# Rongjiehuang/FastDiff

Measured on AMD Instinct MI355X. Metric: real-time factor (audio-sec/wall-sec), N=4 reverse steps, 80x864 mel, higher is better.
Workload: dtype f32 results; 2-piece fp16 operands (22 bit) on fp16 MFMA, fp32 accumulate; GEMM as Winograd F(2,3); exact-fp32 twin; 1 GPU; BASELINE configs[1]: LJSpeech shape, batch=8 x 80x864 mel per GPU, N=4, HIP kernels + hipGraph sampler; batch_per_gpu=8, frames=864, reverse_steps=4, graph=True, weights=random init seed 1234 (no checkpoint offline), world_size=1, gpus_visible=1, oversubscribed=False

## Files before the change

### fastdiff_amd/csrc/fd_api.cpp

```cpp
#include <math.h>
#include <stddef.h>
#include <stdio.h>
#include <stdlib.h>
#include <string.h>

#include <algorithm>

#include "fd_kernels.h"
#include "fd_host.h"

std::string g_create_error;

static inline int gx_rows_host(int T) { return std::max(fdk_fast::gx_rows(T), fdk_fast::gw_pairs(T) * (fdk_fast::GW_ROWB / fdk_fast::GX_ROWB)); }

bool fd_prof_stamps(const fdk::Launch &L, const char *name, hipEvent_t *e0, hipEvent_t *e1)
{
    fd_context *c = L.ctx;
    if (c->profile != 1 || L.capturing) return false;
    hipEvent_t ev[2];
    for (int i = 0; i < 2; ++i) {
        if (!c->event_pool.empty()) { ev[i] = c->event_pool.back(); c->event_pool.pop_back(); }
        else if (hipEventCreate(&ev[i]) != hipSuccess) return false;
    }
    ProfEntry pe;
// ... 730 lines not shown
            int redone = resolve_pending(h, &mask);
            if (redone < 0) return redone;
        }
        if ((rc = copy_out()) != FD_OK) return rc;
    } else {
        if ((rc = enqueue_steps(h, B, T, N, mode, stream)) != FD_OK) return rc;
        if ((rc = copy_out()) != FD_OK) return rc;
    }
    h->last_B = B; h->last_T = T;
    return fd_mark_tail(h, stream);
}

int fd_sample(fd_handle h, const float *mel, int B, int T, const int *lens, const fd_step *table, int N, int ddim,
              const float *x_T, const float *z, uint64_t seed, float *out, float *seq_out, void *stream_)
{
    std::vector<unsigned long long> ids;
    std::vector<long long> offs;
    if (h) { ids.swap(h->noise_ids); offs.swap(h->noise_offs); }
    int rc = check_common(h, B, T, "fd_sample");
    if (rc != FD_OK) return rc;
    if ((rc = fd_follow_stream(h, (hipStream_t)stream_)) != FD_OK) return rc;
    if (h->gen) {
        if (!mel || !table || !out) FD_FAIL(h, FD_ERR_INVALID, "fd_sample: null pointer");
        if (N <= 0 || N > 1024) FD_FAIL(h, FD_ERR_INVALID, "fd_sample: N=%d outside 1..1024", N);
        if (!ids.empty() && (int)ids.size() != B) FD_FAIL(h, FD_ERR_INVALID, "fd_sample: fd_set_noise_streams gave %d stream ids but B=%d", (int)ids.size(), B);
        for (int b = 0; lens && b < B; ++b)
            if (lens[b] < 1 || lens[b] > T) FD_FAIL(h, FD_ERR_INVALID, "fd_sample: lens[%d] = %d outside [1, T=%d]", b, lens[b], T);
        if ((rc = fdg::sample(h, mel, B, T, lens, table, N, ddim, x_T, z, seed, ids, out, seq_out, (hipStream_t)stream_)) != FD_OK) return rc;
        ++h->ticket_counter;
        h->last_B = B; h->last_T = T;
        return fd_mark_tail(h, (hipStream_t)stream_);
    }
    const bool lazy = h->host_fallback && N >= 1 && N <= 8;
    const int Tp = bucket_frames(h, T);
    if ((rc = check_common(h, B, Tp, "fd_sample")) != FD_OK) return rc;
    const int np = (N >= 1 && N <= 1024) ? hoist_mult(h, B, Tp, N) : 1;
    const bool ws_ok = workspace_fits(h, B, Tp, np);
    fd_context::PendingCall prev;
    if (lazy && ws_ok && h->pending.active && h->pending.lazy) {
        prev = h->pending;
        h->pending.active = false;
    } else if ((rc = fd_settle(h)) != FD_OK) return rc;
    auto finish_prev = [&]() -> int {
        if (!prev.active) return FD_OK;
        unsigned mask = 0;
        const fd_context::PendingCall cur = h->pending;
        h->pending.active = false;
        const int r = resolve_call(h, prev, &mask);
        h->pending = cur;
        prev.active = false;
        return r < 0 ? r : FD_OK;
    };
    if (!mel || !table || !out) { finish_prev(); FD_FAIL(h, FD_ERR_INVALID, "fd_sample: null pointer"); }
    if (N <= 0 || N > 1024) { finish_prev(); FD_FAIL(h, FD_ERR_INVALID, "fd_sample: N=%d outside 1..1024", N); }
    if (!ids.empty() && (int)ids.size() != B) {
        finish_prev();
        FD_FAIL(h, FD_ERR_INVALID, "fd_sample: fd_set_noise_streams gave %d stream ids but B=%d", (int)ids.size(), B);
    }
    if (!offs.empty() && offs.size() != ids.size()) { finish_prev(); FD_FAIL(h, FD_ERR_INVALID, "fd_sample: noise offsets without their stream ids"); }
    for (int b = 0; lens && b < B; ++b)
        if (lens[b] < 1 || lens[b] > T) {
            finish_prev();
            FD_FAIL(h, FD_ERR_INVALID, "fd_sample: lens[%d] = %d outside [1, T=%d]", b, lens[b], T);
        }
    if ((rc = ensure_workspace(h, B, Tp, np)) != FD_OK) { finish_prev(); return rc; }
    fd_context::SampleArgs a;
    a.mel = mel; a.B = B; a.T = T; a.N = N; a.ddim = ddim;
    a.has_lens = lens != nullptr;
    if (lens) a.lens.assign(lens, lens + B);
    a.table.assign(table, table + N);
    a.x_T = x_T; a.z = z; a.seed = seed; a.out = out; a.seq_out = seq_out; a.stream = (hipStream_t)stream_;
    a.ids.swap(ids);
    a.offs.swap(offs);
    const long long ticket = ++h->ticket_counter;
    h->n_pieces = h->n_pieces_redone = h->n_pieces_fp32 = 0;
    h->call_fp32_mask = 0;
    rc = sample_core(h, a, 0u, ticket);
    const int rc_prev = finish_prev();
    h->last_B = B; h->last_T = Tp;
    if (rc != FD_OK || rc_prev != FD_OK) return rc != FD_OK ? rc : rc_prev;
    if (!h->defer_check) return fd_settle(h);
    return FD_OK;
}

int64_t fd_sample_ticket(fd_handle h) { return h ? (int64_t)h->ticket_counter : FD_ERR_INVALID; }

static int ticket_redone(fd_handle h, long long ticket)
{
    for (long long t : h->redone_ring)
        if (t == ticket && t != 0) return 1;
    return 0;
}

int fd_sample_settle(fd_handle h, int64_t ticket)
{
    if (!h) return FD_ERR_INVALID;
    if (ticket <= 0 || ticket > h->ticket_counter) FD_FAIL(h, FD_ERR_INVALID, "fd_sample_settle: unknown ticket %lld", (long long)ticket);
    if (h->pending.active && h->pending.ticket <= ticket) {
        FD_HIP(h, hipSetDevice(h->device));
        unsigned mask = 0;
        const int r = resolve_pending(h, &mask);
        if (r < 0) return r;
    }
    return ticket_redone(h, ticket);
}

int fd_sample_check(fd_handle h)
{
    if (!h) return FD_ERR_INVALID;
    if (!h->pending.active) return 0;
    FD_HIP(h, hipSetDevice(h->device));
    unsigned mask = 0;
    return resolve_pending(h, &mask);
}

int fd_set_noise_streams(fd_handle h, const uint64_t *stream_ids, int B)
{
    if (!h || B < 0 || (B > 0 && !stream_ids)) return FD_ERR_INVALID;
    h->noise_ids.assign(stream_ids, stream_ids + B);
    h->noise_offs.clear();
    return FD_OK;
}

int fd_set_option(fd_handle h, const char *key, const char *value)
{
    if (!h || !key || !value) return FD_ERR_INVALID;
    {
        const int rcs = fd_settle(h);
        if (rcs != FD_OK) return rcs;
    }
    const std::string k(key), v(value);
    static const char *stage_names[ST_COUNT] = {"embed", "first", "dblock", "kp_front", "kp_gemm", "convt", "lvc", "final"};
    auto parse_mode = [&](bool &dst) -> int {
        if (v == "fast") dst = true;
        else if (v == "naive") dst = false;
        else FD_FAIL(h, FD_ERR_INVALID, "fd_set_option: %s expects fast|naive, got '%s'", key, value);
        return FD_OK;
    };
    if (k == "kernels") {
        bool m = true;
        int rc = parse_mode(m);
        if (rc != FD_OK) return rc;
        for (int i = 0; i < ST_COUNT; ++i) h->mode.fast[i] = m;
        return FD_OK;
    }
    if (k.compare(0, 8, "kernels.") == 0) {
        for (int i = 0; i < ST_COUNT; ++i)
            if (k.substr(8) == stage_names[i]) return parse_mode(h->mode.fast[i]);
        FD_FAIL(h, FD_ERR_INVALID, "fd_set_option: unknown stage '%s'", key);
    }
    static const struct { const char *key, *a, *b; void (*set)(fd_context *, bool); } choices[] = {
        {"gemm", "f16x2", "fp32", [](fd_context *c, bool a) { c->mode.gemm_f16 = a; }},
        {"gemm_form", "winograd", "direct", [](fd_context *c, bool a) { c->mode.gemm_wino = a; }},
        {"lvc", "f16x2", "fp32", [](fd_context *c, bool a) { c->mode.lvc_f16 = a; }},
        {"conv", "f16x2", "fp32", [](fd_context *c, bool a) { c->mode.conv_f16 = a; }},
        {"lvc_h8", "mfma", "valu", [](fd_context *c, bool a) { c->mode.lvc_h8_mfma = a; }},
        {"fallback", "graph", "host", [](fd_context *c, bool a) { c->host_fallback = !a; }},
        {"lvc_dx", "gather", "copy", [](fd_context *c, bool a) { c->lvc_dx_gather = a; }},
        {"mel", "pwg", "tacotron", [](fd_context *c, bool a) { c->mel_variant = a ? MEL_PWG : MEL_TACOTRON; }},
    };
    for (const auto &ch : choices) {
        if (k != ch.key) continue;
        if (v != ch.a && v != ch.b) FD_FAIL(h, FD_ERR_INVALID, "fd_set_option: %s expects %s|%s, got '%s'", key, ch.a, ch.b, value);
        ch.set(h, v == ch.a);
        return FD_OK;
    }
    const bool on = (v == "1" || v == "true" || v == "on");
    if (k == "fuse_final") { h->mode.fuse_final = on; return FD_OK; }
    if (k == "fuse_up") { h->mode.fuse_up = on; return FD_OK; }
    if (k == "fuse_advance") { h->mode.fuse_advance = on; return FD_OK; }
    if (k == "embed_cache") { h->embed_cache = on; return FD_OK; }
    if (k == "hoist") {
        if (v == "auto") h->hoist_mode = 1;
        else if (v == "on") h->hoist_mode = 2;
        else if (v == "off") h->hoist_mode = 0;
        else FD_FAIL(h, FD_ERR_INVALID, "fd_set_option: hoist expects auto|on|off, got '%s'", value);
        return FD_OK;
    }
    if (k == "graph") { h->use_graph = on; return FD_OK; }
    if (k == "defer_check") { h->defer_check = on; return FD_OK; }
    if (k == "t_bucket" || k == "graph_cache") {
        char *end = nullptr;
        const long n = strtol(value, &end, 10);
        if (end == value || *end != 0 || n < 0 || n > 65536 || (k == "graph_cache" && n < 1))
            FD_FAIL(h, FD_ERR_INVALID, "fd_set_option: %s expects an integer (t_bucket: frames, 0 = exact T; graph_cache: graphs kept, >= 1), got '%s'", key, value);
        if (k == "t_bucket") h->t_bucket = (int)n;
        else h->max_graphs = (int)n;
        return FD_OK;
    }
    if (k == "profile") { h->profile = (v == "events") ? 2 : (on ? 1 : 0); return FD_OK; }
    if (k == "taps") { h->mode.keep_taps = on; return FD_OK; }
    FD_FAIL(h, FD_ERR_INVALID, "fd_set_option: unknown option '%s'", key);
}

}
```

### fastdiff_amd/csrc/fd_internal.h

```cpp
#pragma once
#include <hip/hip_runtime.h>
#include <hip/hip_ext.h>
#include <stdint.h>
#include <string.h>
#include <map>
#include <string>
#include <vector>

#include "../../include/fastdiff_hip.h"
#include "../../include/fastdiff_hip_ext.h"
#include "../../include/fastdiff_hip_train.h"

namespace fd {
constexpr int C = 32;
constexpr int COND = 80;
constexpr int HID = 64;
constexpr int NBLK = 3;
constexpr int LAYERS = 4;
constexpr int HOPT = 256;
constexpr int E_IN = 128, E_MID = 512, E_OUT = 512;
constexpr int KLAYER = 2 * C * C * 3;
constexpr int KW = KLAYER * LAYERS;
constexpr int KB = 2 * C * LAYERS;
constexpr int KREC = KW + KB;
__host__ __device__ constexpr int ratio(int n) { return n == 2 ? 4 : 8; }
__host__ __device__ constexpr int hop(int n) { return n == 0 ? 8 : (n == 1 ? 64 : 256); }
__host__ __device__ constexpr int down_factor(int d) { return d == 0 ? 4 : 8; }

__host__ __device__ inline int kernel_row(int out) { return (out & 15) + 16 * (out >> 5); }
__host__ __device__ inline int kernel_tile(int out) { return (out & 31) >> 4; }
__host__ __device__ inline int kernel_index(int layer, int in, int out, int tap)
{
    const int kk = tap * C + in, kg = kk >> 4, g = (kk >> 3) & 1, e = kk & 7;
    const int mt = kernel_tile(out), lane = kernel_row(out) + 32 * g;
    return layer * KLAYER + ((mt * 6 + kg) * 64 + lane) * 8 + e;
}
__host__ __device__ inline int bias_index(int layer, int out) { return KW + layer * 64 + kernel_tile(out) * 32 + kernel_row(out); }
}

struct ConvW {
    const float *w = nullptr;
    const float *b = nullptr;
};

struct DevWeights {
    ConvW first, final_;
    struct { ConvW res, conv[3]; } down[fd::NBLK];
    struct { ConvW fc_t, up, kp_in, kp_res[6], kc, bc, convs[fd::LAYERS]; } blk[fd::NBLK];
    const float *fc_t1_T = nullptr, *fc_t1_b = nullptr, *fc_t2_T = nullptr, *fc_t2_b = nullptr;
    const float *fc_t_T[fd::NBLK] = {}, *fc_t_b[fd::NBLK] = {};
    const float *embed_table = nullptr;
    const float *down_pack[fd::NBLK][4] = {};
    const uint16_t *down_h2[fd::NBLK][4] = {};
    bool dblock_f16_ok = false;
    const float *lvc_conv_pack[fd::NBLK][fd::LAYERS] = {};
    const uint16_t *lvc_conv_h2[fd::NBLK][fd::LAYERS] = {};
    const uint16_t *lvc_conv_h16[fd::LAYERS] = {};
    bool lvc_f16_ok = false;
    const float *kp_in_pack[fd::NBLK] = {};
    const float *kp_res_pack[fd::NBLK][6] = {};
    const uint16_t *kp_in_h2[fd::NBLK] = {};
    const uint16_t *kp_res_h2[fd::NBLK][6] = {};
    bool kpf_f16_ok = false;
    const float *gemm_pack[fd::NBLK] = {};
    const float *gemm_bias[fd::NBLK] = {};
    const uint16_t *gemm_h2_pack[fd::NBLK] = {};
    bool gemm_f16_ok = false;
    const uint16_t *gemm_w_pack[fd::NBLK] = {};
    bool gemm_w_ok = false;
    const float *up_pack[fd::NBLK] = {};
    const uint16_t *up_h2[fd::NBLK] = {};
    bool convt_f16_ok = false;
    const float *final_fuse = nullptr;
    const int *kc_perm = nullptr;
    const int *bc_perm = nullptr;
};

struct StepParams {
    fd_step table[1024];
    const float *z;
    float *seq;
    unsigned long long seed;
    int n_steps;
    int ddim;
    int step_idx;
    int l4;
    const unsigned long long *uids;
    int l4_io;
    long long n4_io;
    const long long *offs4;
};

enum Stage { ST_EMBED = 0, ST_FIRST, ST_DBLOCK, ST_KP_FRONT, ST_KP_GEMM, ST_CONVT, ST_LVC, ST_FINAL, ST_COUNT };

struct StepMode {
    bool fast[ST_COUNT] = {true, true, true, true, true, true, true, true};
    bool gemm_f16 = true;
    bool gemm_wino = true;
    bool lvc_f16 = true;
    bool conv_f16 = true;
    bool lvc_h8_mfma = true;
    bool fuse_final = true;
    bool fuse_up = true;
    bool fuse_advance = true;
    bool keep_taps = false;
    unsigned fp32_mask = 0;
    bool inline_fallback = true;
    bool ragged = false;
    int hoist_np = 1;
    bool hoist_chunk = false;

    bool operator==(const StepMode &o) const
    {
        for (int i = 0; i < ST_COUNT; ++i)
            if (fast[i] != o.fast[i]) return false;
        return gemm_f16 == o.gemm_f16 && gemm_wino == o.gemm_wino && lvc_f16 == o.lvc_f16 && conv_f16 == o.conv_f16 &&
               lvc_h8_mfma == o.lvc_h8_mfma && fuse_final == o.fuse_final && fuse_up == o.fuse_up && fuse_advance == o.fuse_advance &&
               keep_taps == o.keep_taps && fp32_mask == o.fp32_mask && inline_fallback == o.inline_fallback && ragged == o.ragged &&
               hoist_np == o.hoist_np && hoist_chunk == o.hoist_chunk;
    }
};

struct Workspace {
    int B = 0;
    int64_t frames = 0;
    int64_t rows = 0;
    float *noise = nullptr;
    float *embed_h2 = nullptr;
    float *a[4] = {};
    float *kp_h0 = nullptr, *kp_hA = nullptr, *kp_hB = nullptr;
    float *kpack = nullptr;
    float *h_f16 = nullptr;
    int *lens_dev = nullptr;
    unsigned long long *uid_dev = nullptr;
    long long *off_dev = nullptr;
    float *xsave = nullptr;
    int *range_flag = nullptr;
    float *xA = nullptr, *xB = nullptr;
    float *xtap[fd::NBLK] = {};
    int64_t pframes = 0, prows = 0, plens = 0;
    float *mel_rep = nullptr;
    float *mel = nullptr;
    float *x = nullptr;
    float *eps_acc = nullptr;
    float *steps = nullptr;
    StepParams *params = nullptr;
    size_t bytes = 0;
};

struct ProfEntry { std::string name; hipEvent_t e0, e1; };
struct Scratch { float *p = nullptr; size_t bytes = 0; };

struct MelTables {
    const float *tab = nullptr;
    const int *fb_lo = nullptr, *fb_n = nullptr, *fb_off = nullptr;
    const float *fb_w = nullptr;
};
enum MelVariant { MEL_PWG = 0, MEL_TACOTRON = 1, MEL_VARIANTS = 2 };

struct FoldedParam { std::vector<float> w, b; };
struct WeightImage {
    std::vector<char> bytes;
    std::vector<std::pair<const void **, size_t>> fields;
    template <class T> void add(const T *&dst, const std::vector<T> &v)
    {
        const size_t off = (bytes.size() + 255) & ~(size_t)255;
        bytes.resize(off + v.size() * sizeof(T));
        memcpy(bytes.data() + off, v.data(), v.size() * sizeof(T));
        fields.push_back({reinterpret_cast<const void **>(&dst), off});
    }
};
namespace fdg {
struct Net;
int validate(const fd_config &c, std::string &why);
int create(fd_context *c);
void destroy(fd_context *c);
int hop_total(const fd_context *c);
int pack_weights(fd_context *c, const std::map<std::string, FoldedParam> &f, WeightImage &img);
int forward(fd_context *c, const float *x, const float *mel, const float *steps, int B, int T, const int *lens, float *eps_out, hipStream_t stream);
int sample(fd_context *c, const float *mel, int B, int T, const int *lens, const fd_step *table, int N, int ddim, const float *x_T, const float *z,
           unsigned long long seed, const std::vector<unsigned long long> &ids, float *out, float *seq_out, hipStream_t stream);
}

struct fd_context {
    fd_config cfg;
    fdg::Net *gen = nullptr;
    int device = 0;
    int num_cus = 256;
    std::string err;
    bool committed = false;
    StepMode mode;
    bool use_graph = true;
    int profile = 0;
    std::vector<unsigned long long> noise_ids;
    std::vector<long long> noise_offs;
    bool host_fallback = true;
    std::map<std::string, std::pair<std::vector<int64_t>, std::vector<float>>> raw;
    void *weight_arena = nullptr;
    size_t weight_bytes = 0;
    DevWeights w;
    void *refresh_dev = nullptr;
    size_t refresh_dev_bytes = 0;
    unsigned *refresh_bad = nullptr;
    hipEvent_t refresh_done = nullptr;
    bool refresh_pending = false;
    long long n_refreshes = 0, n_refresh_graph_drops = 0;
    Workspace ws;
    bool lvc_dx_gather = true;
    std::vector<float> embed_t;
    int embed_B = 0;
    bool embed_valid = false;
    bool embed_cache = true;
    MelTables mel[MEL_VARIANTS];
    int mel_variant = MEL_PWG;
    std::vector<float> mel_bank[MEL_VARIANTS];
    bool mel_bank_user[MEL_VARIANTS] = {false, false};
    std::vector<void *> mel_allocs;
    int last_B = 0, last_T = 0;
    hipStream_t cap_stream = nullptr;
    hipStream_t last_stream = nullptr;
    bool have_last_stream = false;
    hipEvent_t ev_switch = nullptr;
    bool tail_marked = false;
    int hoist_mode = 1;
    struct StepGraph { int B, T, steps; StepMode mode; hipGraph_t graph; hipGraphExec_t exec; unsigned long long last_use; };
    std::vector<StepGraph> graphs;
    unsigned long long graph_clock = 0;
    struct RetiredGraph { hipGraph_t graph; hipGraphExec_t exec; hipEvent_t done; };
    std::vector<RetiredGraph> retired;
    int max_graphs = 64;
    int t_bucket = 32;
    long long n_graph_captures = 0, n_graph_hits = 0, n_graph_evictions = 0;
    bool defer_check = false;
    static constexpr int STAGE_SLOTS = 8;
    struct StageSlot { char *host = nullptr; size_t cap = 0; hipEvent_t done = nullptr; };
    StageSlot stage[STAGE_SLOTS];
    unsigned stage_next = 0;
    struct SampleArgs {
        const float *mel = nullptr;
        int B = 0, T = 0, N = 0, ddim = 0;
        bool has_lens = false;
        std::vector<int> lens;
        std::vector<fd_step> table;
        const float *x_T = nullptr, *z = nullptr;
        unsigned long long seed = 0;
        float *out = nullptr, *seq_out = nullptr;
        hipStream_t stream = nullptr;
        std::vector<unsigned long long> ids;
        std::vector<long long> offs;
    };
    struct PendingCall {
        bool active = false;
        bool lazy = false;
        int slot = 0;
        long long ticket = 0;
        int B = 0, T = 0, N = 0, first = 0, count = 0;
        int T_io = 0;
        float *out = nullptr;
        hipStream_t stream = nullptr;
        StepMode mode;
        SampleArgs args;
    } pending;
    long long ticket_counter = 0;
    long long n_pieces = 0, n_pieces_redone = 0, n_pieces_fp32 = 0, n_calls_redone = 0;
    unsigned call_fp32_mask = 0;
    long long redone_ring[16] = {};
    unsigned redone_next = 0;
    int *flags_host = nullptr;
    hipEvent_t flags_done = nullptr, flags_done2 = nullptr;
// ... 104 lines not shown
```

### fastdiff_amd/csrc/fd_kernels.h

```cpp
#pragma once
#include "fd_internal.h"

namespace fdk_fast {
constexpr int GX_CT = 4;
constexpr int GX_ROWB = 2 * 128;
constexpr int GW_PAIRS = 32;
constexpr int GW_ROWB = 1024;
__host__ __device__ inline int gx_rows(int T) { return ((T + GX_CT * 32 - 1) / (GX_CT * 32)) * (GX_CT * 32) + 2; }
__host__ __device__ inline int gw_pairs(int T) { return ((T + 2 * GW_PAIRS - 1) / (2 * GW_PAIRS)) * GW_PAIRS; }
}

namespace fdk {
hipError_t naive_first_conv(const Launch &L, const StepIO &io, int B, int T);
hipError_t naive_dblock(const Launch &L, int d, int B, int T);
hipError_t naive_kp_front(const Launch &L, const StepIO &io, int B, int T);
hipError_t naive_kp_gemm(const Launch &L, int B, int T);
hipError_t naive_convt(const Launch &L, int n, const float *x_in, float *x_out, int B, int Lin);
hipError_t naive_lvc_layer(const Launch &L, int n, int layer, float *x, const float *skip, float *y, int B, int T);
hipError_t naive_final_eps(const Launch &L, const float *x32, float *eps, int B, int T);
hipError_t naive_update(const Launch &L, float *x, const float *eps, int64_t n);
hipError_t fast_first_conv(const Launch &L, const StepIO &io, int B, int T);
hipError_t fast_dblock(const Launch &L, int d, int B, int T, const float *audio);
hipError_t fast_kp_front(const Launch &L, const StepIO &io, int B, int T);
hipError_t fast_kp_gemm(const Launch &L, int B, int T);
hipError_t fast_convt(const Launch &L, int n, const float *x_in, float *x_out, int B, int Lin);
hipError_t fast_lvc_layer(const Launch &L, const StepIO &io, int n, int layer, const float *x_in, const float *skip, float *x_out, int B, int T,
                          bool up = false);
hipError_t fast_final(const Launch &L, const StepIO &io, const float *x32, int B, int T);
bool lvc_op_needs_scratch(int Cin, int Cout, int ks, int hop);
hipError_t lvc_op_forward(const Launch &L, const float *x, const float *K, const float *bias, float *out, int B, int Cin, int Cout, int ks,
                          int T, int hop, float *scratch, int64_t kbs = 0, bool frames = false, int64_t bbs = 0);
hipError_t lvc_op_backward(const Launch &L, const float *x, const float *K, const float *dout, float *dx, float *dK, float *dbias, int B,
                           int Cin, int Cout, int ks, int T, int hop, float *scratch, int64_t kbs = 0, int64_t dkbs = 0, bool frames = false,
                           int64_t dbbs = 0);
hipError_t gate_forward(const Launch &L, const float *x, const float *y, float *out, int B, int C, int64_t len);
hipError_t gate_backward(const Launch &L, const float *y, const float *dout, float *dy, int B, int C, int64_t len);
hipError_t fan_pick(const Launch &L, const float *x, float *out, int rows, int64_t len, int f);
hipError_t fan_sum(const Launch &L, const float *const g[4], const float *gp, float *dx, int rows, int64_t len, int f);
bool kconv_supported(int M, int T);
size_t kconv_scratch_floats(int B, int M, int T);
bool kconv_frames_supported(int M, int T);
bool kconv_act_supported(int M, int T);
hipError_t kconv_forward(const Launch &L, const float *h, const float *W, const float *bias, float *out, int B, int M, int T, bool frames = false,
                         float post = 1.0f);
hipError_t kconv_backward(const Launch &L, const float *h, const float *W, const float *dout, float *dh, float *dW, float *dbias, int B, int M,
                          int T, float *scratch, bool frames = false, const float *y = nullptr, float post = 1.0f, float in_slope = 1.0f);
size_t kconv_w_multi_scratch_floats(int n, int B, int M);
hipError_t kconv_backward_w_multi(const Launch &L, int n, const float *const *h, const float *const *dout, const float *const *y, float post, int B,
                                  int M, int T, float *const *dW, float *const *dbias, float *scratch);
hipError_t kconv_forward_multi(const Launch &L, int n, const float *const *h, const float *const *W, const float *const *bias, float *const *out, int B,
                               int M, int T, float post);
size_t kconv_x_multi_scratch_floats(int n, int B, int M, int T);
hipError_t kconv_backward_x_multi(const Launch &L, int n, const float *const *h, const float *const *W, const float *const *y, const float *const *dout,
                                  float *const *dh, int B, int M, int T, float post, float in_slope, float *scratch);
hipError_t input_conv_forward_multi(const Launch &L, int n, const float *const *x, const float *const *w, const float *const *bias, float *const *out,
                                    int B, int T, float post);
size_t input_conv_multi_scratch_floats(int n, int B);
hipError_t input_conv_backward_multi(const Launch &L, int n, const float *const *x, const float *const *w, const float *const *y, const float *const *dy,
                                     float *const *dx, float *const *dw, float *const *db, int B, int T, float post, float *scratch);
bool cconv_supported(int dil, int64_t len);
size_t cconv_scratch_floats(const Launch &L, int dil, int B, int64_t len);
hipError_t cconv_forward(const Launch &L, const float *x, const float *skip, const float *w, const float *bias, float *xs_out, float *y, int B,
                         int64_t len, int dil, float pre, float post);
hipError_t cconv_backward(const Launch &L, const float *xs, const float *y, const float *w, const float *dy, const float *gxs, float *dxs,
                          float *dw, float *db, int B, int64_t len, int dil, float pre, float post, float *scratch);
size_t conv7_scratch_floats(const Launch &L, int B, int64_t len);
hipError_t conv7_forward(const Launch &L, int which, const float *x, const float *w, const float *bias, float *y, int B, int64_t len);
hipError_t conv7_backward(const Launch &L, int which, const float *x, const float *w, const float *dy, float *dx, float *dw, float *db, int B,
                          int64_t len, float *scratch);
size_t convt_scratch_floats(const Launch &L, int r, int B, int64_t len_in);
hipError_t convt_forward(const Launch &L, const float *x, const float *w, const float *bias, float *y, int B, int64_t len_in, int r);
hipError_t convt_backward(const Launch &L, const float *x, const float *w, const float *dy, float *dx, float *dw, float *db, int B, int64_t len_in,
                          int r, float *scratch);
hipError_t weight_norm_multi(const Launch &L, const fd_wn_item *items, int n, bool backward);
size_t step_scratch_floats(int64_t blocks);
int64_t mse_blocks(int64_t n);
int64_t adamw_blocks(const fd_adamw_item *items, int n);
hipError_t train_draw(const Launch &L, const float *x0, const float *alpha, int T_train, int B, int64_t len, uint64_t seed,
                      const fd_train_state *state, uint64_t iter_host, float *x_t, float *z, float *steps);
hipError_t train_collate(const Launch &L, const float *wav_arena, const float *mel_arena, const int64_t *frame_off, int64_t n_items, int hop,
                         int F, int B, uint64_t seed, const fd_train_state *state, uint64_t iter_host, int rank, int world, float *wavs,
                         float *mels, int64_t *picked);
hipError_t eval_collate(const Launch &L, const float *wav_arena, const float *mel_arena, const int64_t *frame_off, int64_t n_items, int hop,
                        int F, int B, uint64_t seed, const fd_train_state *state, uint64_t iter_host, float *wavs, float *mels, int64_t *picked);
int64_t item_distance_blocks(int64_t n);
hipError_t item_distance(const Launch &L, const float *a, const float *b, int B, int64_t n, int kind, float *out, float *scratch);
hipError_t eval_accumulate(const Launch &L, const float *values, const float *steps, const int64_t *picked, int B, int T_train, int bins,
                           fd_eval_state *acc, float *item_out, fd_train_state *advance);
hipError_t mse_forward(const Launch &L, const float *eps, const float *z, int64_t n, float *loss, fd_train_state *state, float *scratch);
hipError_t mse_backward(const Launch &L, const float *eps, const float *z, const float *dloss, int64_t n, float *deps);
hipError_t adamw_multi(const Launch &L, const fd_adamw_item *items, int n, const fd_adamw_hyper *hyper, fd_train_state *state, float *scratch);
hipError_t ema_multi(const Launch &L, const fd_ema_item *items, int n, const fd_ema_hyper *hyper, const fd_train_state *state, fd_ema_state *ema);
size_t bandpool_scratch_floats(int B, int64_t L, bool backward);
hipError_t bandpool_forward(const Launch &L_, const float *x, const float *W, const float *bias, int B, int64_t L, float *feat, float *scratch);
hipError_t bandpool_backward(const Launch &L_, const float *x, const float *W, const float *bias, const float *dfeat, int B, int64_t L, float *dW,
                             float *db, float *scratch);
hipError_t npred_head_forward(const Launch &L_, const float *feat, const float *beta_next, const float *delta2, int R, const float *W1,
                              const float *b1, const float *W2, const float *b2, int B, float *beta_hat, float *ratio);
hipError_t npred_head_backward(const Launch &L_, const float *feat, const float *beta_next, const float *delta2, const float *W1, const float *b1,
                               const float *W2, const float *b2, const float *dbeta_hat, int B, float *dW1, float *db1, float *dW2, float *db2,
                               float *dfeat);
hipError_t phi_draw(const Launch &L_, const float *x0, const float *alpha, int T_train, int tau, int B, int64_t len, uint64_t seed,
                    const fd_train_state *state, uint64_t iter_host, float *x_t, float *z, float *steps, float *beta_nxt, float *delta,
                    float *delta2);
int64_t phi_residual_blocks(int64_t len);
hipError_t phi_residual_forward(const Launch &L_, const float *eps, const float *z, const float *delta, const float *beta_hat, int B, int64_t len,
                                float *m, float *s, float *scratch);
hipError_t sched_init(const Launch &L_, fd_sched_state *state, float betaN, float alphaN);
hipError_t sched_begin(const Launch &L_, fd_sched_state *state, const float *beta_hat, int n_hat, double rho, const float *alpha, int T_train,
                       int ddim, float *steps_out, int B);
hipError_t sched_update(const Launch &L_, fd_sched_state *state, float *x, const float *eps, int64_t n, float *cond_out);
}

namespace fdg {
struct ConvArgs {
    const float *x, *w, *bias;
    float *y;
    int B, Cin, Cout, K;
    int64_t Lx, Lout;
    int dil = 1, in_stride = 1;
    float pre = 1.0f, post = 1.0f;
    const float *in_add = nullptr;
    int64_t in_add_b = 0, in_add_step = 0;
    const int *step = nullptr;
    const float *res = nullptr;
    const int *lens = nullptr;
    int spf = 1;
    int rec = 0, rec_off = 0;
    const int *perm = nullptr;
    ConvArgs(const ConvW &cw, const float *x_, float *y_, int B_, int Cin_, int Cout_, int K_, int64_t L)
        : x(x_), w(cw.w), bias(cw.b), y(y_), B(B_), Cin(Cin_), Cout(Cout_), K(K_), Lx(L), Lout(L) {}
};
hipError_t conv1d(const fdk::Launch &L, const char *name, const ConvArgs &a);
hipError_t convt(const fdk::Launch &L, const char *name, const ConvW &up, const float *x, float *y, int B, int C, int r, int64_t Lin,
                 const int *lens, int spf_in);
hipError_t dblock(const fdk::Launch &L, const ConvW &res, const ConvW conv[3], const float *x, int64_t Lin, int f, float *const tmp[3],
                  float *out, int B, int C, const int *lens, int spf);
hipError_t kp_front(const fdk::Launch &L, const ConvArgs &in, const ConvW res[6], int k, float *ha, float *hb);
struct LvcArgs {
    float *x;
    const float *skip;
    float *y;
    bool packed;
    const float *kernels, *biases;
    int B, C, ks, layers, layer, hop, T;
    const int *lens;
};
hipError_t lvc_layer(const fdk::Launch &L, const ConvW &conv, const LvcArgs &a);
}
```

### fastdiff_amd/csrc/fd_kernels_kp.hip

```cpp
#include "fd_kernels_common.h"

namespace fdk_fast {

constexpr int KPF_VALID = 48, KPF_LDI = 68, KPF_LDH = 66;

struct KpFrontW {
    const float *in_pack[fd::NBLK], *in_b[fd::NBLK];
    const float *res_pack[fd::NBLK][6], *res_b[fd::NBLK][6];
};

__global__ void __launch_bounds__(256, 2) k_kp_front(const float *__restrict__ mel, float *__restrict__ hout, KpFrontW w,
                                                     const float *__restrict__ noise, const StepParams *params, int sampler,
                                                     int B, int T, const int *__restrict__ run_if, const int *__restrict__ lens)
{
    __shared__ float xin[fd::COND * KPF_LDI];
    if (run_if && *run_if == 0) return;
    __shared__ float h0[fd::HID * KPF_LDH];
    __shared__ float hA[fd::HID * KPF_LDH];
    __shared__ float hB[fd::HID * KPF_LDH];
    const int blk = blockIdx.z, b = blockIdx.y, t0 = blockIdx.x * KPF_VALID;
    const int Tb = frames_of(lens, b, T);
    if (t0 >= Tb) return;
    const int tid = threadIdx.x, lane = tid & 63, wave = tid >> 6, l31 = lane & 31, hi = lane >> 5;
    const int mt = wave & 1, nt = wave >> 1;
// ... 600 lines not shown
                have_blk = cur.blk; have_xg = cur.xg;
                __builtin_amdgcn_s_waitcnt(0x0F70);
            }
            const bool more = (i + half + 1 < n_mine);
            GX_WALK_NEXT(walk, cur, more, nxt, run, left);
            const int Tb = frames_of(lens, cur.b, T);
            const bool full = (Tb % 32 == 0) || (cur.chunk * (GX_CT * 32) + GX_CT * 32 <= Tb);
            if (half == 0) {
                if (full) gx_item<0, true>(lds, cur, more, nxt, hx, kpack, wq, bias_lo, aoff, B, T, R, wave_u, lane, Tb GX_TIMING_PASS);
                else gx_item<0, false>(lds, cur, more, nxt, hx, kpack, wq, bias_lo, aoff, B, T, R, wave_u, lane, Tb GX_TIMING_PASS);
            } else {
                if (full) gx_item<1, true>(lds, cur, more, nxt, hx, kpack, wq, bias_lo, aoff, B, T, R, wave_u, lane, Tb GX_TIMING_PASS);
                else gx_item<1, false>(lds, cur, more, nxt, hx, kpack, wq, bias_lo, aoff, B, T, R, wave_u, lane, Tb GX_TIMING_PASS);
            }
            cur = nxt;
        }
    }
#ifdef FD_GX_TIMING
    ph[6] = __builtin_amdgcn_s_memtime() - t_start;
    ph[7] = __builtin_amdgcn_s_memrealtime() - r_start;
    if (lane == 0)
        for (int k = 0; k < 8; ++k) atomicAdd((unsigned long long *)&fd_gxdbg[k], (unsigned long long)ph[k]);
#endif
}

constexpr int GW_WINB = GW_PAIRS * GW_ROWB;

__global__ void __launch_bounds__(256) k_h_wino(const float *__restrict__ h, char *__restrict__ wx, int *__restrict__ range_flag, int B, int T,
                                                int P, const int *__restrict__ lens)
{
    const int bb = blockIdx.y;
    const int e = blockIdx.x * 256 + threadIdx.x, p = e >> 3, g = e & 7;
    if (p >= P) return;
    if (range_flag[32] != 0) {
        if (e == 0 && bb == 0) atomicOr(range_flag, 1);
        return;
    }
    const int Tb = frames_of(lens, bb % B, T);
    const float *hb = h + ((int64_t)bb * fd::HID + 8 * g) * T;
    const int t1 = 2 * p;
    float d[8][4];
#pragma unroll
    for (int c = 0; c < 8; ++c) {
        const float *hc = hb + (int64_t)c * T;
        d[c][0] = (t1 - 1 >= 0 && t1 - 1 < Tb) ? hc[t1 - 1] : 0.0f;
        d[c][1] = (t1 < Tb) ? hc[t1] : 0.0f;
        d[c][2] = (t1 + 1 < Tb) ? hc[t1 + 1] : 0.0f;
        d[c][3] = (t1 + 2 < Tb) ? hc[t1 + 2] : 0.0f;
    }
    float mx = 0.0f;
    char *row = wx + ((int64_t)bb * P + p) * GW_ROWB;
    const int sw = p & 15;
#pragma unroll
    for (int j = 0; j < 4; ++j) {
        float u[8];
#pragma unroll
        for (int c = 0; c < 8; ++c) {
            u[c] = j == 0 ? d[c][0] - d[c][2] : (j == 1 ? d[c][1] + d[c][2] : (j == 2 ? d[c][2] - d[c][1] : d[c][1] - d[c][3]));
            mx = fmaxf(mx, fabsf(u[c]));
        }
        float4 ph, pl;
        split8(u, ph, pl);
        *reinterpret_cast<float4 *>(row + j * 256 + ((g ^ sw) << 4)) = ph;
        *reinterpret_cast<float4 *>(row + j * 256 + (((g + 8) ^ sw) << 4)) = pl;
    }
    if (!(mx < GX_LIMIT)) atomicOr(range_flag, 1);
}

__device__ __forceinline__ void gw_dma(const char *wx, char *lds_buf, const GxItem &it, int B, int P, int wave_u, int lane)
{
#ifndef FD_GW_NO_FETCH
    gx_window_dma<GW_WINB / 4096, false>(wx + (((int64_t)it.blk * B + it.b) * P + it.chunk * GW_PAIRS) * GW_ROWB + wave_u * 1024, lds_buf, wave_u, lane);
#endif
}

template <int BUF, bool FULL>
__device__ __forceinline__ void gw_item(char *lds, const GxItem &cur, bool more, const GxItem &nxt, const char *wx, float *kpack,
                                        const float4 (&wq)[2][16], float bias_lo, const int (&aoff)[2][4], int B, int T, int P,
                                        int wave_u, int lane, int Tb)
{
    const int l31 = lane & 31, hi = lane >> 5;
    if (more) gw_dma(wx, lds + (BUF ^ 1) * GW_WINB, nxt, B, P, wave_u, lane);
    const int t_begin = cur.chunk * (2 * GW_PAIRS);
    float *krow = kpack + (((int64_t)cur.blk * B + cur.b) * T + t_begin) * fd::KREC + (cur.xg * 4 + wave_u) * 32;
    const unsigned loff = (unsigned)(8 * hi) * (unsigned)fd::KREC + (unsigned)l31;
    const __amdgpu_buffer_rsrc_t rs = __builtin_amdgcn_make_buffer_rsrc(krow, 0, 2 * GW_PAIRS * fd::KREC * 4, 0x00020000);
    const f32x16 zero = {0.f, 0.f, 0.f, 0.f, 0.f, 0.f, 0.f, 0.f, 0.f, 0.f, 0.f, 0.f, 0.f, 0.f, 0.f, 0.f};
    const char *hb = lds + BUF * GW_WINB;
    constexpr int ORDER[4] = {1, 2, 0, 3};
    f32x16 keep, acc, lo;
#pragma unroll
    for (int r = 0; r < 16; ++r) lo[r] = bias_lo;
    float4 a1, a2;
    auto store16 = [&](int odd) {
#ifdef FD_GX_NO_STORE
        if (FULL) {
#pragma unroll
            for (int r = 0; r < 16; ++r) { const float v_ = fmaf(lo[r], GX_INV_SCALE, acc[r]); asm volatile("" :: "v"(v_)); }
            (void)rs; (void)loff;
            return;
        }
#endif
        if (FULL) {
#pragma unroll
            for (int r = 0; r < 16; ++r) {
                acc[r] = fmaf(lo[r], GX_INV_SCALE, acc[r]);
                __builtin_amdgcn_raw_buffer_store_b32(__float_as_uint(acc[r]), rs, loff * 4u, (2 * ((r & 3) + 8 * (r >> 2)) + odd) * fd::KREC * 4,
                                                      FD_GX_STORE_AUX);
            }
        } else {
#pragma unroll
            for (int r = 0; r < 16; ++r)
                if (t_begin + 2 * drow(r, hi) + odd < Tb) (krow + (2 * ((r & 3) + 8 * (r >> 2)) + odd) * fd::KREC)[loff] = fmaf(lo[r], GX_INV_SCALE, acc[r]);
        }
    };
#pragma unroll
    for (int s = 0; s < 4; ++s) {
        const int j = ORDER[s];
        a1 = *reinterpret_cast<const float4 *>(hb + aoff[0][0] + j * 256);
        a2 = *reinterpret_cast<const float4 *>(hb + aoff[1][0] + j * 256);
#pragma unroll
        for (int k4 = 0; k4 < 4; ++k4) {
            const int kg = j * 4 + k4;
            float4 n1 = a1, n2 = a2;
            if (k4 + 1 < 4) {
                n1 = *reinterpret_cast<const float4 *>(hb + aoff[0][k4 + 1] + j * 256);
                n2 = *reinterpret_cast<const float4 *>(hb + aoff[1][k4 + 1] + j * 256);
            }
            acc = mfma_f16(a1, wq[0][kg], (k4 == 0 && s == 0) ? zero : ((k4 == 0 && s == 3) ? keep : acc));
            lo = mfma_f16(a2, wq[0][kg], (k4 == 0 && s == 3) ? zero : lo);
            lo = mfma_f16(a1, wq[1][kg], lo);
            a1 = n1;
            a2 = n2;
        }
        if (s == 0) {
#pragma unroll
            for (int r = 0; r < 16; ++r) keep[r] = fmaf(lo[r], GX_INV_SCALE, acc[r]);
        } else if (s == 1) {
#pragma unroll
            for (int r = 0; r < 16; ++r) keep[r] = fmaf(2.0f, keep[r], -fmaf(lo[r], GX_INV_SCALE, acc[r]));
        } else store16(s == 3 ? 1 : 0);
    }
    if (more) {
#ifdef FD_GX_NO_STORE
        asm volatile("s_waitcnt vmcnt(0)" ::: "memory");
#else
        if (FULL) asm volatile("s_waitcnt vmcnt(32)" ::: "memory");
        else asm volatile("s_waitcnt vmcnt(0)" ::: "memory");
#endif
    }
    __builtin_amdgcn_s_barrier();
}

__global__ void __launch_bounds__(256, 2) k_kp_gemm_w(const char *__restrict__ wx , float *__restrict__ kpack,
                                                      const float4 *g0, const float4 *g1, const float4 *g2, const float *gb0,
                                                      const float *gb1, const float *gb2, const int *__restrict__ range_flag, int B,
                                                      int T, int P, int chunks_per_utt, int n_items, const int *__restrict__ lens)
{
    __shared__ __attribute__((aligned(16))) char lds[2 * GW_WINB];
    const int tid = threadIdx.x, lane = tid & 63, l31 = lane & 31, hi = lane >> 5;
    const int wave_u = __builtin_amdgcn_readfirstlane(tid >> 6);
    if (*range_flag != 0) return;
    GxWalk walk(B, chunks_per_utt, n_items, gridDim.x, blockIdx.x);
    const int n_mine = walk.n_mine;
    if (n_mine <= 0) return;
    int run = 0, left = walk.left0;
    GxItem cur = walk.first();
    int aoff[2][4];
#pragma unroll
    for (int q2 = 0; q2 < 2; ++q2)
#pragma unroll
        for (int k4 = 0; k4 < 4; ++k4) aoff[q2][k4] = l31 * GW_ROWB + (((q2 * 8 + k4 * 2 + hi) ^ (l31 & 15)) << 4);
    gw_dma(wx, lds, cur, B, P, wave_u, lane);
    asm volatile("s_waitcnt vmcnt(0)" ::: "memory");
    __builtin_amdgcn_s_barrier();
    float4 wq[2][16];
    float bias_lo = 0.0f;
    int have_blk = -1, have_xg = -1;
#pragma unroll 1
    for (int i = 0; i < n_mine; i += 2) {
#pragma unroll
        for (int half = 0; half < 2; ++half) {
            if (half == 1 && i + 1 >= n_mine) break;
            if (cur.blk != have_blk || cur.xg != have_xg) {
                const float4 *gp = cur.blk == 0 ? g0 : (cur.blk == 1 ? g1 : g2);
                const float *gb = cur.blk == 0 ? gb0 : (cur.blk == 1 ? gb1 : gb2);
                const int ptile = cur.xg * 4 + wave_u;
#pragma unroll
                for (int q2 = 0; q2 < 2; ++q2)
#pragma unroll
                    for (int kg = 0; kg < 16; ++kg) wq[q2][kg] = gp[(((int64_t)ptile * 2 + q2) * 16 + kg) * 64 + lane];
                bias_lo = gb[ptile * 32 + l31] * GX_SCALE;
                have_blk = cur.blk; have_xg = cur.xg;
                __builtin_amdgcn_s_waitcnt(0x0F70);
            }
            const bool more = (i + half + 1 < n_mine);
            GX_WALK_NEXT(walk, cur, more, nxt, run, left);
            const int Tb = frames_of(lens, cur.b, T);
            const bool full = cur.chunk * (2 * GW_PAIRS) + 2 * GW_PAIRS <= Tb;
            if (half == 0) {
                if (full) gw_item<0, true>(lds, cur, more, nxt, wx, kpack, wq, bias_lo, aoff, B, T, P, wave_u, lane, Tb);
                else gw_item<0, false>(lds, cur, more, nxt, wx, kpack, wq, bias_lo, aoff, B, T, P, wave_u, lane, Tb);
            } else {
                if (full) gw_item<1, true>(lds, cur, more, nxt, wx, kpack, wq, bias_lo, aoff, B, T, P, wave_u, lane, Tb);
                else gw_item<1, false>(lds, cur, more, nxt, wx, kpack, wq, bias_lo, aoff, B, T, P, wave_u, lane, Tb);
            }
            cur = nxt;
        }
    }
}

}

namespace fdk {
using namespace fdk_fast;

hipError_t fast_kp_front(const Launch &L, const StepIO &io, int B, int T)
{
    fd_context *c = L.ctx;
    const DevWeights &w = c->w;
    const dim3 grid((T + KPF_VALID - 1) / KPF_VALID, B, fd::NBLK);
    const StepMode &m = *L.mode;
    const int *lens = m.ragged ? c->ws.lens_dev : nullptr;
    const int *run_if = nullptr;
    const char *name = "kp_front";
    const Pipe pipe = fd_pipe(m, m.conv_f16 && w.kpf_f16_ok, 19);
    if (pipe != PIPE_F32_ONLY) {
        KpFrontW2 k2;
        for (int n = 0; n < fd::NBLK; ++n) {
            k2.in_pack[n] = reinterpret_cast<const float4 *>(w.kp_in_h2[n]); k2.in_b[n] = w.blk[n].kp_in.b;
            for (int l = 0; l < 6; ++l) { k2.res_pack[n][l] = reinterpret_cast<const float4 *>(w.kp_res_h2[n][l]); k2.res_b[n][l] = w.blk[n].kp_res[l].b; }
        }
        const bool image = front_writes_h_image(m, w);
        FD_LAUNCH(L, name, k_kp_front_h2, grid, dim3(256), 0, io.mel, c->ws.kp_hB, image ? reinterpret_cast<char *>(c->ws.h_f16) : (char *)nullptr, k2,
                  (const float *)c->ws.noise, (const StepParams *)c->ws.params, io.sampler, B, T, gx_rows(T), c->ws.range_flag, lens);
        run_if = c->ws.range_flag + 19;
        name = "kp_front_fp32_fallback";
        if (pipe == PIPE_F16_ONLY) return hipSuccess;
    }
    KpFrontW kw;
    for (int n = 0; n < fd::NBLK; ++n) {
        kw.in_pack[n] = w.kp_in_pack[n]; kw.in_b[n] = w.blk[n].kp_in.b;
        for (int l = 0; l < 6; ++l) { kw.res_pack[n][l] = w.kp_res_pack[n][l]; kw.res_b[n][l] = w.blk[n].kp_res[l].b; }
    }
    FD_LAUNCH(L, name, k_kp_front, grid, dim3(256), 0, io.mel, c->ws.kp_hB, kw, (const float *)c->ws.noise,
              (const StepParams *)c->ws.params, io.sampler, B, T, run_if, lens);
    return hipSuccess;
}

struct GemmGrid { int chunks, items, grid; };
static GemmGrid gemm_grid(const fd_context *c, int B, int chunks)
{
    const int items = fd::NBLK * (fd::KREC / 128) * B * chunks;
    return {chunks, items, items < 2 * c->num_cus ? items : 2 * c->num_cus};
}

hipError_t fast_kp_gemm(const Launch &L, int B, int T)
{
    fd_context *c = L.ctx;
    const DevWeights &w = c->w;
    const StepMode &m = *L.mode;
    const int *lens = m.ragged ? c->ws.lens_dev : nullptr;
    const Pipe pipe = fd_pipe(m, m.gemm_f16 && w.gemm_f16_ok, 0);
    const bool f16 = pipe != PIPE_F32_ONLY;
    if (f16 && m.gemm_wino && w.gemm_w_ok) {
        const int P = gw_pairs(T);
        const GemmGrid g = gemm_grid(c, B, P / GW_PAIRS);
        FD_LAUNCH(L, "h_wino", k_h_wino, dim3((8 * P + 255) / 256, fd::NBLK * B), dim3(256), 0, (const float *)c->ws.kp_hB,
                  reinterpret_cast<char *>(c->ws.h_f16), c->ws.range_flag, B, T, P, lens);
        FD_LAUNCH(L, "kp_gemm_f16x2", k_kp_gemm_w, dim3(g.grid), dim3(256), 0, reinterpret_cast<const char *>(c->ws.h_f16), c->ws.kpack,
                  reinterpret_cast<const float4 *>(w.gemm_w_pack[0]), reinterpret_cast<const float4 *>(w.gemm_w_pack[1]),
                  reinterpret_cast<const float4 *>(w.gemm_w_pack[2]), w.gemm_bias[0], w.gemm_bias[1], w.gemm_bias[2],
                  (const int *)c->ws.range_flag, B, T, P, g.chunks, g.items, lens);
        if (pipe == PIPE_F16_ONLY) return hipSuccess;
    } else if (f16) {
        const int R = gx_rows(T);
        const GemmGrid g = gemm_grid(c, B, (T + GX_CT * 32 - 1) / (GX_CT * 32));
        if (!front_writes_h_image(m, w))
            FD_LAUNCH(L, "h_split", k_h_split, dim3((32 * R + 255) / 256, fd::NBLK * B), dim3(256), 0, (const float *)c->ws.kp_hB,
                      reinterpret_cast<unsigned *>(c->ws.h_f16), c->ws.range_flag, B, T, R, lens);
        FD_LAUNCH(L, "kp_gemm_f16x2", k_kp_gemm_h2, dim3(g.grid), dim3(256), 0, reinterpret_cast<const char *>(c->ws.h_f16), c->ws.kpack,
                  reinterpret_cast<const float4 *>(w.gemm_h2_pack[0]), reinterpret_cast<const float4 *>(w.gemm_h2_pack[1]),
                  reinterpret_cast<const float4 *>(w.gemm_h2_pack[2]), w.gemm_bias[0], w.gemm_bias[1], w.gemm_bias[2],
                  (const int *)c->ws.range_flag, B, T, R, g.chunks, g.items, lens);
        if (pipe == PIPE_F16_ONLY) return hipSuccess;
    }
    const int tiles_per_utt = (T + 31) / 32;
    const GemmGrid g = gemm_grid(c, B, (tiles_per_utt + GEMM_CT - 1) / GEMM_CT);
    const int chunk_tiles = (tiles_per_utt + g.chunks - 1) / g.chunks;
    FD_LAUNCH(L, f16 ? "kp_gemm_fp32_fallback" : "kp_gemm", k_kp_gemm, dim3(g.grid), dim3(256), 0, (const float *)c->ws.kp_hB, c->ws.kpack,
              w.gemm_pack[0], w.gemm_pack[1], w.gemm_pack[2], w.gemm_bias[0], w.gemm_bias[1], w.gemm_bias[2], B, T, g.chunks,
              chunk_tiles, g.items, f16 ? (const int *)c->ws.range_flag : (const int *)nullptr, lens);
    return hipSuccess;
}

}
```

Before: 9979 x real-time.

## Add 16x16x32 MFMA tile variant of Winograd kernel-predictor GEMM

Adds a 16-row MFMA tile path (mfma_f32_16x16x32_f16) for the Winograd F(2,3) kernel-predictor GEMM, with new LDS addressing, a weight register layout, permlane16_swap-based buffer stores and adjusted vmcnt waits. It becomes the default through a new gemm_tile option, and the 32-row path stays selectable. The aim is higher MFMA throughput and finer tail handling for ragged lengths. The cost is a different register and LDS access pattern plus new indexing code that has to match the packed weight layout.

After: 10180 x real-time (median of 6 runs). +2.0%, better.

```diff
diff --git a/fastdiff_amd/csrc/fd_api.cpp b/fastdiff_amd/csrc/fd_api.cpp
--- a/fastdiff_amd/csrc/fd_api.cpp
+++ b/fastdiff_amd/csrc/fd_api.cpp
@@ -906,6 +906,7 @@
     static const struct { const char *key, *a, *b; void (*set)(fd_context *, bool); } choices[] = {
         {"gemm", "f16x2", "fp32", [](fd_context *c, bool a) { c->mode.gemm_f16 = a; }},
         {"gemm_form", "winograd", "direct", [](fd_context *c, bool a) { c->mode.gemm_wino = a; }},
+        {"gemm_tile", "16", "32", [](fd_context *c, bool a) { c->mode.gemm_tile16 = a; }},
         {"lvc", "f16x2", "fp32", [](fd_context *c, bool a) { c->mode.lvc_f16 = a; }},
         {"conv", "f16x2", "fp32", [](fd_context *c, bool a) { c->mode.conv_f16 = a; }},
         {"lvc_h8", "mfma", "valu", [](fd_context *c, bool a) { c->mode.lvc_h8_mfma = a; }},
diff --git a/fastdiff_amd/csrc/fd_internal.h b/fastdiff_amd/csrc/fd_internal.h
--- a/fastdiff_amd/csrc/fd_internal.h
+++ b/fastdiff_amd/csrc/fd_internal.h
@@ -97,6 +97,7 @@
     bool fast[ST_COUNT] = {true, true, true, true, true, true, true, true};
     bool gemm_f16 = true;
     bool gemm_wino = true;
+    bool gemm_tile16 = true;
     bool lvc_f16 = true;
     bool conv_f16 = true;
     bool lvc_h8_mfma = true;
@@ -114,7 +115,7 @@
     {
         for (int i = 0; i < ST_COUNT; ++i)
             if (fast[i] != o.fast[i]) return false;
-        return gemm_f16 == o.gemm_f16 && gemm_wino == o.gemm_wino && lvc_f16 == o.lvc_f16 && conv_f16 == o.conv_f16 &&
+        return gemm_f16 == o.gemm_f16 && gemm_wino == o.gemm_wino && gemm_tile16 == o.gemm_tile16 && lvc_f16 == o.lvc_f16 && conv_f16 == o.conv_f16 &&
                lvc_h8_mfma == o.lvc_h8_mfma && fuse_final == o.fuse_final && fuse_up == o.fuse_up && fuse_advance == o.fuse_advance &&
                keep_taps == o.keep_taps && fp32_mask == o.fp32_mask && inline_fallback == o.inline_fallback && ragged == o.ragged &&
                hoist_np == o.hoist_np && hoist_chunk == o.hoist_chunk;
diff --git a/fastdiff_amd/csrc/fd_kernels.h b/fastdiff_amd/csrc/fd_kernels.h
--- a/fastdiff_amd/csrc/fd_kernels.h
+++ b/fastdiff_amd/csrc/fd_kernels.h
@@ -8,6 +8,21 @@
 constexpr int GW_ROWB = 1024;
 __host__ __device__ inline int gx_rows(int T) { return ((T + GX_CT * 32 - 1) / (GX_CT * 32)) * (GX_CT * 32) + 2; }
 __host__ __device__ inline int gw_pairs(int T) { return ((T + 2 * GW_PAIRS - 1) / (2 * GW_PAIRS)) * GW_PAIRS; }
+
+__host__ __device__ inline int gw16_a_off(int lane, int q, int ks)
+{
+    const int r = lane & 15, g = lane >> 4;
+    return r * GW_ROWB + (((8 * q + 4 * ks + g) ^ r) << 4);
+}
+__host__ __device__ inline int gw16_b_idx(int ptile, int q, int j, int ks, int ct, int lane)
+{
+    const int kh = 4 * ks + (lane >> 4);
+    return ((ptile * 2 + q) * 16 + 4 * j + (kh >> 1)) * 64 + 32 * (kh & 1) + 16 * ct + (lane & 15);
+}
+__host__ __device__ inline int gw16_d_pair(int lane, int i) { return 4 * (lane >> 4) + i; }
+__host__ __device__ inline int gw16_d_pos(int lane, int ct) { return 16 * ct + (lane & 15); }
+__host__ __device__ inline unsigned gw16_st_lane_off(int lane) { return (unsigned)(16 * (lane >> 5)) * (unsigned)fd::KREC + (unsigned)(lane & 31); }
+__host__ __device__ inline int gw16_st_row_off(int rt, int part, int i, int odd) { return (2 * (16 * rt + 4 * part + i) + odd) * fd::KREC; }
 }
 
 namespace fdk {
diff --git a/fastdiff_amd/csrc/fd_kernels_kp.hip b/fastdiff_amd/csrc/fd_kernels_kp.hip
--- a/fastdiff_amd/csrc/fd_kernels_kp.hip
+++ b/fastdiff_amd/csrc/fd_kernels_kp.hip
@@ -776,11 +776,122 @@
     __builtin_amdgcn_s_barrier();
 }
 
+typedef float gw_f4 __attribute__((ext_vector_type(4)));
+__device__ __forceinline__ gw_f4 mfma16_f16(const float4 &a, const float4 &b, gw_f4 c)
+{
+    union { float4 f; f16x8 h; } ua, ub;
+    ua.f = a;
+    ub.f = b;
+    return __builtin_amdgcn_mfma_f32_16x16x32_f16(ua.h, ub.h, c, 0, 0, 0);
+}
+template <int BUF>
+__device__ __forceinline__ void gw16_item(char *lds, const GxItem &cur, bool more, const GxItem &nxt, const char *wx, float *kpack,
+                                          const float4 (&wq)[2][16] , const float (&bias_lo)[2],
+                                          const int (&aoff)[2][2], int B, int T, int P, int wave_u, int lane, int Tb)
+{
+    if (more) gw_dma(wx, lds + (BUF ^ 1) * GW_WINB, nxt, B, P, wave_u, lane);
+    const int t_begin = cur.chunk * (2 * GW_PAIRS);
+    float *krow = kpack + (((int64_t)cur.blk * B + cur.b) * T + t_begin) * fd::KREC + (cur.xg * 4 + wave_u) * 32;
+    const unsigned loff = gw16_st_lane_off(lane);
+    const __amdgpu_buffer_rsrc_t rs = __builtin_amdgcn_make_buffer_rsrc(krow, 0, 2 * GW_PAIRS * fd::KREC * 4, 0x00020000);
+    const gw_f4 zero = {0.f, 0.f, 0.f, 0.f};
+    constexpr int ORDER[4] = {1, 2, 0, 3};
+    int n_fast = 0;
+    bool counted = true;
+#pragma unroll
+    for (int rt = 0; rt < 2; ++rt) {
+        const int t0 = t_begin + 32 * rt;
+        if (t0 >= Tb) continue;
+        const bool whole = t0 + 32 <= Tb;
+        const char *hb = lds + BUF * GW_WINB + rt * 16 * GW_ROWB;
+        gw_f4 acc[2], lo[2], keep[2];
+#pragma unroll
+        for (int ct = 0; ct < 2; ++ct) lo[ct] = gw_f4{bias_lo[ct], bias_lo[ct], bias_lo[ct], bias_lo[ct]};
+        float4 a1 = *reinterpret_cast<const float4 *>(hb + aoff[0][0] + ORDER[0] * 256);
+        float4 a2 = *reinterpret_cast<const float4 *>(hb + aoff[1][0] + ORDER[0] * 256);
+#ifdef FD_GW16_PIN
+        __builtin_amdgcn_sched_group_barrier(0x100, 2, 0);
+#endif
+#pragma unroll
+        for (int step = 0; step < 8; ++step) {
+            const int s = step >> 1, ks = step & 1, j = ORDER[s], w = (2 * j + ks) * 2;
+            float4 n1 = a1, n2 = a2;
+            if (step + 1 < 8) {
+                const int jn = ORDER[(step + 1) >> 1], kn = (step + 1) & 1;
+                n1 = *reinterpret_cast<const float4 *>(hb + aoff[0][kn] + jn * 256);
+                n2 = *reinterpret_cast<const float4 *>(hb + aoff[1][kn] + jn * 256);
+            }
+            const bool m3 = (step == 6);
+            acc[0] = mfma16_f16(a1, wq[0][w], step == 0 ? zero : (m3 ? keep[0] : acc[0]));
+            lo[0] = mfma16_f16(a2, wq[0][w], m3 ? zero : lo[0]);
+            acc[1] = mfma16_f16(a1, wq[0][w + 1], step == 0 ? zero : (m3 ? keep[1] : acc[1]));
+            lo[1] = mfma16_f16(a2, wq[0][w + 1], m3 ? zero : lo[1]);
+            lo[0] = mfma16_f16(a1, wq[1][w], lo[0]);
+            lo[1] = mfma16_f16(a1, wq[1][w + 1], lo[1]);
+            a1 = n1;
+            a2 = n2;
+#ifdef FD_GW16_PIN
+            if (step + 1 < 8) __builtin_amdgcn_sched_group_barrier(0x100, 2, 0);
+            __builtin_amdgcn_sched_group_barrier(0x008, 6, 0);
+#endif
+            if (ks == 0) continue;
+            if (s == 0) {
+#pragma unroll
+                for (int ct = 0; ct < 2; ++ct)
+#pragma unroll
+                    for (int i = 0; i < 4; ++i) keep[ct][i] = fmaf(lo[ct][i], GX_INV_SCALE, acc[ct][i]);
+            } else if (s == 1) {
+#pragma unroll
+                for (int ct = 0; ct < 2; ++ct)
+#pragma unroll
+                    for (int i = 0; i < 4; ++i) keep[ct][i] = fmaf(2.0f, keep[ct][i], -fmaf(lo[ct][i], GX_INV_SCALE, acc[ct][i]));
+            } else {
+                const int odd = s == 3 ? 1 : 0;
+                float v[2][4];
+#pragma unroll
+                for (int ct = 0; ct < 2; ++ct)
+#pragma unroll
+                    for (int i = 0; i < 4; ++i) v[ct][i] = fmaf(lo[ct][i], GX_INV_SCALE, acc[ct][i]);
+                if (whole) {
+#pragma unroll
+                    for (int i = 0; i < 4; ++i) {
+                        const auto x = __builtin_amdgcn_permlane16_swap(__float_as_uint(v[0][i]), __float_as_uint(v[1][i]), false, false);
+#pragma unroll
+                        for (int part = 0; part < 2; ++part)
+                            __builtin_amdgcn_raw_buffer_store_b32(x[part], rs, loff * 4u, gw16_st_row_off(rt, part, i, odd) * 4, FD_GX_STORE_AUX);
+                    }
+                } else {
+#pragma unroll
+                    for (int ct = 0; ct < 2; ++ct)
+#pragma unroll
+                        for (int i = 0; i < 4; ++i) {
+                            const int f = 2 * (16 * rt + gw16_d_pair(lane, i)) + odd;
+                            if (t_begin + f < Tb) krow[f * fd::KREC + gw16_d_pos(lane, ct)] = v[ct][i];
+                        }
+                }
+            }
+        }
+        if (whole) ++n_fast;
+        else counted = false;
+    }
+    if (more) {
+        if (counted && n_fast == 2) asm volatile("s_waitcnt vmcnt(32)" ::: "memory");
+        else if (counted && n_fast == 1) asm volatile("s_waitcnt vmcnt(16)" ::: "memory");
+        else asm volatile("s_waitcnt vmcnt(0)" ::: "memory");
+    }
+    __builtin_amdgcn_s_barrier();
+}
+
+#ifdef FD_GW_CLOCK
+__device__ long long fd_gwclk[2];
+#endif
+template <int TILE>
 __global__ void __launch_bounds__(256, 2) k_kp_gemm_w(const char *__restrict__ wx , float *__restrict__ kpack,
                                                       const float4 *g0, const float4 *g1, const float4 *g2, const float *gb0,
                                                       const float *gb1, const float *gb2, const int *__restrict__ range_flag, int B,
                                                       int T, int P, int chunks_per_utt, int n_items, const int *__restrict__ lens)
 {
+    static_assert(TILE == 16 || TILE == 32, "k_kp_gemm_w: 16- or 32-row matrix tiles");
     __shared__ __attribute__((aligned(16))) char lds[2 * GW_WINB];
     const int tid = threadIdx.x, lane = tid & 63, l31 = lane & 31, hi = lane >> 5;
     const int wave_u = __builtin_amdgcn_readfirstlane(tid >> 6);
@@ -790,16 +901,21 @@
     if (n_mine <= 0) return;
     int run = 0, left = walk.left0;
     GxItem cur = walk.first();
-    int aoff[2][4];
+    constexpr int NOFF = TILE == 16 ? 2 : 4;
+    int aoff[2][NOFF];
 #pragma unroll
     for (int q2 = 0; q2 < 2; ++q2)
 #pragma unroll
-        for (int k4 = 0; k4 < 4; ++k4) aoff[q2][k4] = l31 * GW_ROWB + (((q2 * 8 + k4 * 2 + hi) ^ (l31 & 15)) << 4);
+        for (int k4 = 0; k4 < NOFF; ++k4)
+            aoff[q2][k4] = TILE == 16 ? gw16_a_off(lane, q2, k4) : l31 * GW_ROWB + (((q2 * 8 + k4 * 2 + hi) ^ (l31 & 15)) << 4);
     gw_dma(wx, lds, cur, B, P, wave_u, lane);
     asm volatile("s_waitcnt vmcnt(0)" ::: "memory");
     __builtin_amdgcn_s_barrier();
+#ifdef FD_GW_CLOCK
+    const long long clk_t0 = __builtin_amdgcn_s_memtime(), clk_r0 = __builtin_amdgcn_s_memrealtime();
+#endif
     float4 wq[2][16];
-    float bias_lo = 0.0f;
+    float bias_lo[2] = {0.0f, 0.0f};
     int have_blk = -1, have_xg = -1;
 #pragma unroll 1
     for (int i = 0; i < n_mine; i += 2) {
@@ -810,28 +926,50 @@
                 const float4 *gp = cur.blk == 0 ? g0 : (cur.blk == 1 ? g1 : g2);
                 const float *gb = cur.blk == 0 ? gb0 : (cur.blk == 1 ? gb1 : gb2);
                 const int ptile = cur.xg * 4 + wave_u;
-#pragma unroll
-                for (int q2 = 0; q2 < 2; ++q2)
-#pragma unroll
-                    for (int kg = 0; kg < 16; ++kg) wq[q2][kg] = gp[(((int64_t)ptile * 2 + q2) * 16 + kg) * 64 + lane];
-                bias_lo = gb[ptile * 32 + l31] * GX_SCALE;
+                if constexpr (TILE == 16) {
+#pragma unroll
+                    for (int q2 = 0; q2 < 2; ++q2)
+#pragma unroll
+                        for (int jk = 0; jk < 8; ++jk)
+#pragma unroll
+                            for (int ct = 0; ct < 2; ++ct) wq[q2][jk * 2 + ct] = gp[gw16_b_idx(ptile, q2, jk >> 1, jk & 1, ct, lane)];
+#pragma unroll
+                    for (int ct = 0; ct < 2; ++ct) bias_lo[ct] = gb[ptile * 32 + gw16_d_pos(lane, ct)] * GX_SCALE;
+                } else {
+#pragma unroll
+                    for (int q2 = 0; q2 < 2; ++q2)
+#pragma unroll
+                        for (int kg = 0; kg < 16; ++kg) wq[q2][kg] = gp[(((int64_t)ptile * 2 + q2) * 16 + kg) * 64 + lane];
+                    bias_lo[0] = gb[ptile * 32 + l31] * GX_SCALE;
+                }
                 have_blk = cur.blk; have_xg = cur.xg;
                 __builtin_amdgcn_s_waitcnt(0x0F70);
             }
             const bool more = (i + half + 1 < n_mine);
             GX_WALK_NEXT(walk, cur, more, nxt, run, left);
             const int Tb = frames_of(lens, cur.b, T);
-            const bool full = cur.chunk * (2 * GW_PAIRS) + 2 * GW_PAIRS <= Tb;
-            if (half == 0) {
-                if (full) gw_item<0, true>(lds, cur, more, nxt, wx, kpack, wq, bias_lo, aoff, B, T, P, wave_u, lane, Tb);
-                else gw_item<0, false>(lds, cur, more, nxt, wx, kpack, wq, bias_lo, aoff, B, T, P, wave_u, lane, Tb);
+            if constexpr (TILE == 16) {
+                if (half == 0) gw16_item<0>(lds, cur, more, nxt, wx, kpack, wq, bias_lo, aoff, B, T, P, wave_u, lane, Tb);
+                else gw16_item<1>(lds, cur, more, nxt, wx, kpack, wq, bias_lo, aoff, B, T, P, wave_u, lane, Tb);
             } else {
-                if (full) gw_item<1, true>(lds, cur, more, nxt, wx, kpack, wq, bias_lo, aoff, B, T, P, wave_u, lane, Tb);
-                else gw_item<1, false>(lds, cur, more, nxt, wx, kpack, wq, bias_lo, aoff, B, T, P, wave_u, lane, Tb);
+                const bool full = cur.chunk * (2 * GW_PAIRS) + 2 * GW_PAIRS <= Tb;
+                if (half == 0) {
+                    if (full) gw_item<0, true>(lds, cur, more, nxt, wx, kpack, wq, bias_lo[0], aoff, B, T, P, wave_u, lane, Tb);
+                    else gw_item<0, false>(lds, cur, more, nxt, wx, kpack, wq, bias_lo[0], aoff, B, T, P, wave_u, lane, Tb);
+                } else {
+                    if (full) gw_item<1, true>(lds, cur, more, nxt, wx, kpack, wq, bias_lo[0], aoff, B, T, P, wave_u, lane, Tb);
+                    else gw_item<1, false>(lds, cur, more, nxt, wx, kpack, wq, bias_lo[0], aoff, B, T, P, wave_u, lane, Tb);
+                }
             }
             cur = nxt;
         }
     }
+#ifdef FD_GW_CLOCK
+    if (tid == 0) {
+        atomicAdd((unsigned long long *)&fd_gwclk[0], (unsigned long long)(__builtin_amdgcn_s_memtime() - clk_t0));
+        atomicAdd((unsigned long long *)&fd_gwclk[1], (unsigned long long)(__builtin_amdgcn_s_memrealtime() - clk_r0));
+    }
+#endif
 }
 
 }
@@ -892,7 +1030,9 @@
         const GemmGrid g = gemm_grid(c, B, P / GW_PAIRS);
         FD_LAUNCH(L, "h_wino", k_h_wino, dim3((8 * P + 255) / 256, fd::NBLK * B), dim3(256), 0, (const float *)c->ws.kp_hB,
                   reinterpret_cast<char *>(c->ws.h_f16), c->ws.range_flag, B, T, P, lens);
-        FD_LAUNCH(L, "kp_gemm_f16x2", k_kp_gemm_w, dim3(g.grid), dim3(256), 0, reinterpret_cast<const char *>(c->ws.h_f16), c->ws.kpack,
+        const auto gemm_w = m.gemm_tile16 ? &k_kp_gemm_w<16> : &k_kp_gemm_w<32>;
+        FD_LAUNCH(L, "kp_gemm_f16x2", gemm_w, dim3(g.grid), dim3(256), 0,
+                  reinterpret_cast<const char *>(c->ws.h_f16), c->ws.kpack,
                   reinterpret_cast<const float4 *>(w.gemm_w_pack[0]), reinterpret_cast<const float4 *>(w.gemm_w_pack[1]),
                   reinterpret_cast<const float4 *>(w.gemm_w_pack[2]), w.gemm_bias[0], w.gemm_bias[1], w.gemm_bias[2],
                   (const int *)c->ws.range_flag, B, T, P, g.chunks, g.items, lens);
```
